# facebookresearch/metamorph

Measured on AMD Instinct MI355X. Metric: train tokens/sec (LLaMA-3-8B + SigLIP-SO400M, seq2048, 256 img toks), whole job, higher is better.
Workload: dtype bf16

## Files before the change

### include/mm355.h

```cpp
#ifndef MM355_H
#define MM355_H

#include <stddef.h>
#include <stdint.h>

#ifdef __cplusplus
extern "C" {
#endif

#define MM355_VERSION 100

#define MM355_OK            0
#define MM355_EINVAL       -1
#define MM355_EUNSUPPORTED -2
#define MM355_ELAUNCH      -3

typedef uint16_t mm355_bf16;

int mm355_version(void);
const char* mm355_strerror(int code);

#define MM355_GEMM_BIAS        1u
#define MM355_GEMM_GELU_ERF    2u
#define MM355_GEMM_GELU_TANH   4u
// ... 28 lines not shown
int mm355_gemm_rope_bf16(const mm355_bf16* X, int64_t ldx, const mm355_bf16* Wqkv, int64_t ldw, mm355_bf16* qkv, int64_t ld_qkv,
                         const mm355_bf16* cos_t, const mm355_bf16* sin_t, const int32_t* pos_offset,
                         int64_t M, int64_t N, int64_t K, int64_t L, int64_t n_rot, void* stream);

int mm355_gemm_swiglu_bwd_bf16(const mm355_bf16* dY, int64_t ldy, const mm355_bf16* WdT, int64_t ldw, const mm355_bf16* gu, int64_t ld_gu,
                               mm355_bf16* dgu, int64_t ld_dgu, mm355_bf16* actT, mm355_bf16* dguT, int64_t ldT,
                               int64_t M, int64_t I, int64_t K, void* stream);

int mm355_gemm_pair_bf16(const mm355_bf16* A0, int64_t lda0, const mm355_bf16* B0, int64_t ldb0, void* C0, int64_t ldc0,
                         int64_t M0, int64_t N0, int64_t K0, uint32_t flags0,
                         const mm355_bf16* A1, int64_t lda1, const mm355_bf16* B1, int64_t ldb1, void* C1, int64_t ldc1,
                         int64_t M1, int64_t N1, int64_t K1, uint32_t flags1, void* stream);

int mm355_transpose_bf16(const mm355_bf16* in, int64_t ld_in, int64_t rows, int64_t cols,
                         mm355_bf16* out, int64_t ld_out, void* stream);

int mm355_colsum_bf16(const mm355_bf16* dY, int64_t ld, int64_t M, int64_t N, float* db_f32, void* stream);

int mm355_rmsnorm_fwd(const mm355_bf16* x, const mm355_bf16* w, mm355_bf16* y, int64_t M, int64_t h,
                      float eps, void* stream);
int mm355_rmsnorm_fwd_rstd(const mm355_bf16* x, const mm355_bf16* w, mm355_bf16* y, float* rstd_out, int64_t M, int64_t h,
                           float eps, void* stream);
int mm355_rmsnorm_apply_t(const mm355_bf16* x, const mm355_bf16* w, const float* rstd, int64_t M, int64_t h,
                          mm355_bf16* out_t, int64_t ld_out, void* stream);
int mm355_rmsnorm_bwd(const mm355_bf16* dy, const mm355_bf16* x, const mm355_bf16* w,
                      const mm355_bf16* dres, mm355_bf16* dx, float* dw_f32, float* workspace,
                      int64_t M, int64_t h, float eps, void* stream);
int64_t mm355_rmsnorm_bwd_ws_floats(int64_t M, int64_t h);
int mm355_rmsnorm_bwd_wgrad(const mm355_bf16* dy, const mm355_bf16* x, const mm355_bf16* w, const mm355_bf16* dres,
                            mm355_bf16* dx, mm355_bf16* w_grad, int accumulate, float* workspace,
// ... 82 lines not shown
int mm355_swiglu_bwd_t(const mm355_bf16* gu, const mm355_bf16* dact, mm355_bf16* dgu, mm355_bf16* actT,
                       mm355_bf16* dguT, int64_t M, int64_t I, void* stream);
#define MM355_GELU_ERF  0
#define MM355_GELU_TANH 1
int mm355_gelu_fwd(const mm355_bf16* x, mm355_bf16* y, int64_t n, int kind, void* stream);
int mm355_gelu_bwd(const mm355_bf16* x, const mm355_bf16* dy, mm355_bf16* dx, int64_t n, int kind, void* stream);
int mm355_scale_bf16(mm355_bf16* x, int64_t n, const float* s_dev, float s_host, void* stream);
int mm355_axpy_bf16(mm355_bf16* y, const mm355_bf16* x, int64_t n, const float* s_dev, float s_host,
                    int accumulate, void* stream);
int mm355_axpy_f32_to_bf16(mm355_bf16* y, const float* x, int64_t n, float s_host, int accumulate, void* stream);
int mm355_axpy_f32_to_bf16_dev(mm355_bf16* y, const float* x, int64_t n, const float* s_dev, float s_host, int accumulate,
                               void* stream);

int mm355_ce_rows(mm355_bf16* logits, int64_t ld, const int32_t* targets, int64_t R, int64_t V,
                  float grad_scale, float* loss_sum, float* row_ws, void* stream);
int mm355_sum_rows_f32(const float* values, int64_t n, float scale, float* out, int accumulate, void* stream);

int64_t mm355_linear_ce_ws_bytes(int64_t n, int64_t V, int64_t h, int gather, int need_dh, int need_dw);
int mm355_linear_ce(const mm355_bf16* hidden, int64_t ldh, const int32_t* rows, const int32_t* targets, int64_t n,
                    const mm355_bf16* W, int64_t ldw, int64_t V, int64_t h, float* loss, mm355_bf16* d_hidden, void* dW,
                    int dw_f32, void* workspace, int64_t workspace_bytes, void* stream);

int mm355_splice_gather(const mm355_bf16* embed, const mm355_bf16* proj, const int32_t* src,
                        mm355_bf16* out, int64_t rows, int64_t h, void* stream);
int mm355_rows_gather(const mm355_bf16* in, int64_t ld_in, const int32_t* idx, mm355_bf16* out, int64_t ld_out,
                      int64_t R, int64_t h, void* stream);
int mm355_rows_scatter_add(const mm355_bf16* src, int64_t ld_src, const int32_t* idx, mm355_bf16* dst,
                           int64_t ld_dst, int64_t R, int64_t h, void* stream);
int mm355_embed_grad(const mm355_bf16* dout, const int32_t* tok, const int32_t* seg_start, const int32_t* pos,
                     int64_t n_seg, mm355_bf16* dembed, int64_t h, int accumulate, void* stream);
// ... 31 lines not shown
```

### metamorph_amd/csrc/gemm_bf16.hip

```cpp
#include "gemm_common.h"
#include <type_traits>
#include <cstdlib>

namespace {

template <int TM, int TN, int FM, int FN>
MM_DEV void gemm_epilogue(f32x4 (&acc)[FM][FN], const GemmArgs& a, unsigned char* smem, int m0, int n0, int wm, int wn, int wave, int lane) {
    const int fr = lane & 15, fq = lane >> 4;
    const int M = a.M, N = a.N;
    constexpr int CPL = TN / 4;
    float* stg = (float*)smem + wave * (16 * TN);
    const uint32_t fl = a.flags;
    const int row_l = lane >> 2, col_l = (lane & 3) * CPL;
    uint16_t* Cb = (uint16_t*)a.C;
    float* Cf = (float*)a.C;
    const bool vec_ok = ((a.ldc & 7) == 0) && (!(fl & MM355_GEMM_RESIDUAL) || (a.ldr & 7) == 0);
#pragma unroll
    for (int i = 0; i < FM; ++i) {
        __builtin_amdgcn_fence(__ATOMIC_RELEASE, "wavefront");
        __builtin_amdgcn_wave_barrier();
#pragma unroll
        for (int j = 0; j < FN; ++j)
#pragma unroll
            for (int r = 0; r < 4; ++r) stg[(fq * 4 + r) * TN + j * 16 + fr] = acc[i][j][r];
        __builtin_amdgcn_fence(__ATOMIC_RELEASE, "wavefront");
        __builtin_amdgcn_wave_barrier();
        const int grow = m0 + wm * TM + i * 16 + row_l;
        if (grow < M) {
            const int64_t rr = (fl & MM355_GEMM_RESIDUAL) ? (a.res_mod > 0 ? (int64_t)(grow % a.res_mod) : (int64_t)grow) : 0;
#pragma unroll
            for (int j = 0; j < CPL / 8; ++j) {
                const int c = n0 + wn * TN + col_l + j * 8;
                if (c >= N) continue;
                float v[8];
                const f32x4 s0 = *(const f32x4*)(stg + row_l * TN + col_l + j * 8);
                const f32x4 s1 = *(const f32x4*)(stg + row_l * TN + col_l + j * 8 + 4);
                v[0] = s0.x; v[1] = s0.y; v[2] = s0.z; v[3] = s0.w;
                v[4] = s1.x; v[5] = s1.y; v[6] = s1.z; v[7] = s1.w;
                epi_store8(a, fl, vec_ok, grow, rr, c, v);
            }
        }
    }
}

MM_DEV void gemm_epilogue_swiglu(f32x4 (&acc)[8][4], const GemmArgs& a, unsigned char* smem, int m0, int tn, int wm, int wn, int wave, int lane) {
    constexpr int TN = 64;
    const int fr = lane & 15, fq = lane >> 4;
    const int M = a.M, I = (int)a.res_mod;
    float* stg = (float*)smem + wave * (16 * TN);
    const int row_l = lane >> 2, k4 = lane & 3;
    uint16_t* gu = (uint16_t*)a.C;
    uint16_t* act = (uint16_t*)a.res;
    const int ch0 = tn * 128 + wn * 32;
#pragma unroll
// ... 383 lines not shown

template <int N> MM_DEV void wait_vmcnt() {
#if defined(MM355_SWB_ABL) && MM355_SWB_ABL == 3
    static_assert(N >= 0 && N <= 10, "unsupported count");
    asm volatile("s_waitcnt vmcnt(%0)" :: "n"(N) : "memory");
#else
    static_assert(N == 0 || N == 2 || N == 4 || N == 6 || N == 8, "unsupported count");
    if constexpr (N == 8) asm volatile("s_waitcnt vmcnt(8)" ::: "memory");
    else if constexpr (N == 6) asm volatile("s_waitcnt vmcnt(6)" ::: "memory");
    else if constexpr (N == 4) asm volatile("s_waitcnt vmcnt(4)" ::: "memory");
    else if constexpr (N == 2) asm volatile("s_waitcnt vmcnt(2)" ::: "memory");
    else asm volatile("s_waitcnt vmcnt(0)" ::: "memory");
#endif
}

template <int ABL = 0, bool SWI = false, bool SWB = false, bool ROPE = false>
MM_DEV void gemm_pp_tile(const GemmArgs& a, const int bid, unsigned char* smem) {
    constexpr int BM = 256, BN = 256, TM = 128, TN = 64, FM = 8, FN = 4;
    constexpr int BUF = (BM + BN) * 128;
    constexpr int A_BYTES = BM * 128;

    const int total = a.ntm * a.ntn;
    const int q8 = total >> 3, r8 = total & 7;
    const int xcd = bid & 7, idx = bid >> 3;
    const int logical = (xcd < r8 ? xcd * (q8 + 1) : r8 * (q8 + 1) + (xcd - r8) * q8) + idx;
    const int GM = a.gm;
    const int gsize = GM * a.ntn;
    const int grp = logical / gsize;
    const int first_m = grp * GM;
    const int gm = min(a.ntm - first_m, GM);
    const int in_g = logical - grp * gsize;
// ... 201 lines not shown
    __syncthreads();
#if defined(MM355_SWB_ABL) && (MM355_SWB_ABL == 1 || MM355_SWB_ABL == 3)
    if constexpr (SWB) {
        float keep = 0.f;
#pragma unroll
        for (int i = 0; i < FM; ++i)
#pragma unroll
            for (int j = 0; j < FN; ++j) keep += acc[i][j][0] + acc[i][j][1] + acc[i][j][2] + acc[i][j][3];
        if (keep == 1.2345e-30f) ((float*)a.C)[tid] = keep;
        return;
    }
#endif
    if constexpr (SWI) gemm_epilogue_swiglu(acc, a, smem, m0, tn, wm, wn, wave, lane);
    else if constexpr (SWB) gemm_epilogue_swiglu_bwd(acc, a, smem, m0, n0, wm, wn, wave, lane);
    else if constexpr (ROPE) gemm_epilogue_rope(acc, a, smem, m0, n0, wm, wn, wave, lane);
    else gemm_epilogue<TM, TN, FM, FN>(acc, a, smem, m0, n0, wm, wn, wave, lane);
}

__global__ __launch_bounds__(512) void gemm_pp_swiglu_kernel(GemmArgs a) {
    extern __shared__ __attribute__((aligned(16))) unsigned char smem[];
    gemm_pp_tile<0, true>(a, blockIdx.x, smem);
}

__global__ __launch_bounds__(512) void gemm_pp_rope_kernel(GemmArgs a) {
    extern __shared__ __attribute__((aligned(16))) unsigned char smem[];
    gemm_pp_tile<0, false, false, true>(a, blockIdx.x, smem);
}

__global__ __launch_bounds__(512) void gemm_pp_swiglu_bwd_kernel(GemmArgs a) {
    extern __shared__ __attribute__((aligned(16))) unsigned char smem[];
    gemm_pp_tile<0, false, true>(a, blockIdx.x, smem);
// ... 71 lines not shown
int launch_gemm(GemmArgs a, hipStream_t s) {
    constexpr int STAGE = (BM + BN) * 128;
    constexpr int LDS = 2 * STAGE;
    auto kern = gemm_nt_kernel<BM, BN, WM, WN, GLDS, PIPE>;
    static std::atomic<uint64_t> lds_ok{0};
    if (mm_ensure_dynamic_lds((const void*)kern, LDS, lds_ok) != MM355_OK) return MM355_ELAUNCH;
    a.ntm = (a.M + BM - 1) / BM;
    a.ntn = (a.N + BN - 1) / BN;
    const int64_t total = (int64_t)a.ntm * a.ntn;
    if (total <= 0 || total > 0x7fffffff) return MM355_EINVAL;
    hipLaunchKernelGGL(kern, dim3((unsigned)total), dim3(WM * WN * 64), LDS, s, a);
    return mm_launch_status();
}

__global__ __launch_bounds__(256) void transpose_kernel(const uint16_t* __restrict__ in, int64_t ld_in, int rows, int cols,
                                                        uint16_t* __restrict__ out, int64_t ld_out) {
    __shared__ uint16_t tile[64][64 + 2];
    const int r0 = blockIdx.y * 64, c0 = blockIdx.x * 64;
    const int tid = threadIdx.x;
#pragma unroll
    for (int i = 0; i < 2; ++i) {
        const int v = tid + i * 256, r = v >> 3, c = (v & 7) * 8;
        const int gr = r0 + r, gc = c0 + c;
        uint16_t tmp[8];
        if (gr < rows && gc + 8 <= cols) {
            *(u32x4*)tmp = *(const u32x4*)(in + (int64_t)gr * ld_in + gc);
        } else {
#pragma unroll
            for (int e = 0; e < 8; ++e) tmp[e] = (gr < rows && gc + e < cols) ? in[(int64_t)gr * ld_in + gc + e] : (uint16_t)0;
        }
#pragma unroll
        for (int e = 0; e < 8; ++e) tile[r][c + e] = tmp[e];
    }
    __syncthreads();
#pragma unroll
    for (int i = 0; i < 2; ++i) {
        const int v = tid + i * 256, c = v >> 3, r = (v & 7) * 8;
        const int gc = c0 + c, gr = r0 + r;
        if (gc >= cols) continue;
        uint16_t tmp[8];
#pragma unroll
        for (int e = 0; e < 8; ++e) tmp[e] = tile[r + e][c];
        if (gr + 8 <= rows && ((ld_out & 7) == 0)) {
            *(u32x4*)(out + (int64_t)gc * ld_out + gr) = *(const u32x4*)tmp;
        } else {
            for (int e = 0; e < 8; ++e)
                if (gr + e < rows) out[(int64_t)gc * ld_out + gr + e] = tmp[e];
        }
    }
}

__global__ __launch_bounds__(256) void colsum_kernel(const uint16_t* __restrict__ x, int64_t ld, int M, int N, float* __restrict__ out) {
    __shared__ float part[4][64];
    const int cq = threadIdx.x & 63, rp = threadIdx.x >> 6;
    const int c = blockIdx.x * 64 + cq;
    float s = 0.f;
    if (c < N)
        for (int r = rp; r < M; r += 4) s += bf2f(x[(int64_t)r * ld + c]);
    part[rp][cq] = s;
    __syncthreads();
    if (rp == 0 && c < N) out[c] += (part[0][cq] + part[1][cq]) + (part[2][cq] + part[3][cq]);
}
// ... 371 lines not shown
}

extern "C" int mm355_gemm_pair_bf16(const mm355_bf16* A0, int64_t lda0, const mm355_bf16* B0, int64_t ldb0, void* C0, int64_t ldc0,
                                    int64_t M0, int64_t N0, int64_t K0, uint32_t flags0,
                                    const mm355_bf16* A1, int64_t lda1, const mm355_bf16* B1, int64_t ldb1, void* C1, int64_t ldc1,
                                    int64_t M1, int64_t N1, int64_t K1, uint32_t flags1, void* stream) {
    (void)hipGetLastError();
    GemmArgs a0, a1;
    int rc = pair_problem(a0, A0, lda0, B0, ldb0, C0, ldc0, M0, N0, K0, flags0);
    if (rc != MM355_OK) return rc;
    rc = pair_problem(a1, A1, lda1, B1, ldb1, C1, ldc1, M1, N1, K1, flags1);
    if (rc != MM355_OK) return rc;
    return launch_gemm_pp_pair(a0, a1, (hipStream_t)stream);
}

extern "C" int mm355_transpose_bf16(const mm355_bf16* in, int64_t ld_in, int64_t rows, int64_t cols, mm355_bf16* out,
                                    int64_t ld_out, void* stream) {
    (void)hipGetLastError();
    if (!in || !out || rows <= 0 || cols <= 0 || (ld_in & 7) || !mm_aligned16(in) || !mm_aligned16(out)) return MM355_EINVAL;
    if (ld_out < rows || rows > 0x7fffffff || cols > 0x7fffffff) return MM355_EINVAL;
    dim3 grid((unsigned)((cols + 63) / 64), (unsigned)((rows + 63) / 64));
    hipLaunchKernelGGL(transpose_kernel, grid, dim3(256), 0, (hipStream_t)stream, in, ld_in, (int)rows, (int)cols, out, ld_out);
    return mm_launch_status();
}

extern "C" int mm355_gemm_swiglu_bf16(const mm355_bf16* X, int64_t ldx, const mm355_bf16* Wgu, int64_t ldw, mm355_bf16* gu, int64_t ld_gu,
                                      mm355_bf16* act, int64_t ld_act, int64_t M, int64_t I, int64_t K, void* stream) {
    (void)hipGetLastError();
    if (!X || !Wgu || !gu || !act || M <= 0 || I <= 0 || K <= 0) return MM355_EINVAL;
    if ((ldx & 7) || (ldw & 7) || (ld_gu & 7) || (ld_act & 7) || !mm_aligned16(X) || !mm_aligned16(Wgu) || !mm_aligned16(gu) || !mm_aligned16(act))
        return MM355_EINVAL;
    if (M > 0x7fffffff || I > 0x3fffffff || K > 0x7fffffff) return MM355_EINVAL;
    if ((I & 127) || K < 128 || (K & 127) || (2 * I * ldw + K) * 2 >= 0x7fffffffLL || (256 * ldx + K) * 2 >= 0x7fffffffLL) return MM355_EUNSUPPORTED;
    GemmArgs a = {};
    a.A = X; a.B = Wgu; a.C = gu; a.bias = nullptr; a.res = act;
    a.lda = ldx; a.ldb = ldw; a.ldc = ld_gu; a.ldr = ld_act; a.res_mod = I;
    a.M = (int)M; a.N = (int)(2 * I); a.K = (int)K; a.flags = 0; a.ntm = a.ntn = 0;
// ... 64 lines not shown
```

### metamorph_amd/csrc/linear_ce.hip

```cpp
#include "mm355_common.h"

#include <algorithm>

namespace {

constexpr int64_t CE_CHUNK = 8192;

inline int64_t up(int64_t x, int64_t a) { return (x + a - 1) / a * a; }
inline int64_t padded_rows(int64_t R) { return R >= 512 ? up(R, 128) : up(R, 8); }

struct Layout {
    int64_t Vp, chunk, rp, hc, wt, logits, dyT, xT, rows, total;
};

Layout layout(int64_t n, int64_t V, int64_t h, int gather, int need_dh, int need_dw) {
    Layout l{};
    l.Vp = up(V, 128);
    l.chunk = std::min(n, CE_CHUNK);
    l.rp = padded_rows(l.chunk);
    int64_t off = 0;
    auto take = [&](int64_t bytes) { const int64_t o = off; off += up(bytes, 256); return o; };
    l.hc = gather ? take(n * h * 2) : -1;
    l.wt = need_dh ? take(h * l.Vp * 2) : -1;
    l.logits = take(l.chunk * l.Vp * 2);
    l.dyT = need_dw ? take(V * l.rp * 2) : -1;
    l.xT = need_dw ? take(h * l.rp * 2) : -1;
    l.rows = take(n * 4);
    l.total = off;
    return l;
}

}

extern "C" int64_t mm355_linear_ce_ws_bytes(int64_t n, int64_t V, int64_t h, int gather, int need_dh, int need_dw) {
    if (n <= 0 || V <= 0 || h <= 0) return 0;
    return layout(n, V, h, gather, need_dh, need_dw).total;
}

extern "C" int mm355_linear_ce(const mm355_bf16* hidden, int64_t ldh, const int32_t* rows, const int32_t* targets, int64_t n,
                               const mm355_bf16* W, int64_t ldw, int64_t V, int64_t h, float* loss, mm355_bf16* d_hidden, void* dW,
                               int dw_f32, void* workspace, int64_t workspace_bytes, void* stream) {
    if (!hidden || !targets || !W || !loss || !workspace || n <= 0 || V <= 0 || h <= 0 || (h & 7) || (ldh & 7) || (ldw & 7) || ldh < h || ldw < h ||
        n > 0x7fffffff || !mm_aligned16(workspace))
        return MM355_EINVAL;
    const int need_dh = d_hidden != nullptr, need_dw = dW != nullptr, gather = rows != nullptr;
    const Layout l = layout(n, V, h, gather, need_dh, need_dw);
    if (workspace_bytes < l.total) return MM355_EINVAL;
    hipStream_t s = (hipStream_t)stream;
    char* ws = (char*)workspace;
    const mm355_bf16* hc = hidden;
    int64_t ldc = ldh;
    int rc;
    if (gather) {
        mm355_bf16* g = (mm355_bf16*)(ws + l.hc);
        if ((rc = mm355_rows_gather(hidden, ldh, rows, g, h, n, h, stream)) != MM355_OK) return rc;
        hc = g;
        ldc = h;
    }
    mm355_bf16* wt = need_dh ? (mm355_bf16*)(ws + l.wt) : nullptr;
    if (need_dh) {
        if (l.Vp != V && hipMemset2DAsync(wt + V, l.Vp * 2, 0, (l.Vp - V) * 2, h, s) != hipSuccess) return MM355_ELAUNCH;
        if ((rc = mm355_transpose_bf16(W, ldw, V, h, wt, l.Vp, stream)) != MM355_OK) return rc;
    }
    mm355_bf16* logits = (mm355_bf16*)(ws + l.logits);
    float* row_nll = (float*)(ws + l.rows);
    const float inv = 1.0f / (float)n;
    bool first = true;
    for (int64_t r0 = 0; r0 < n; r0 += CE_CHUNK) {
        const int64_t r = std::min(n - r0, CE_CHUNK);
        const mm355_bf16* x = hc + r0 * ldc;
        if ((rc = mm355_gemm_bf16(x, ldc, W, ldw, logits, l.Vp, r, V, h, nullptr, nullptr, 0, 0, 0u, 0, stream)) != MM355_OK) return rc;
        if ((rc = mm355_ce_rows(logits, l.Vp, targets + r0, r, V, inv, nullptr, row_nll + r0, stream)) != MM355_OK) return rc;
        if (need_dh &&
            (rc = mm355_gemm_bf16(logits, l.Vp, wt, l.Vp, d_hidden + r0 * h, h, r, h, l.Vp, nullptr, nullptr, 0, 0, 0u, 0, stream)) != MM355_OK)
            return rc;
        if (need_dw) {
            const int64_t rp = padded_rows(r);
            mm355_bf16* dyT = (mm355_bf16*)(ws + l.dyT);
            mm355_bf16* xT = (mm355_bf16*)(ws + l.xT);
            if (rp != r) {
                if (hipMemset2DAsync(dyT + r, rp * 2, 0, (rp - r) * 2, V, s) != hipSuccess) return MM355_ELAUNCH;
                if (hipMemset2DAsync(xT + r, rp * 2, 0, (rp - r) * 2, h, s) != hipSuccess) return MM355_ELAUNCH;
            }
            if ((rc = mm355_transpose_bf16(logits, l.Vp, r, V, dyT, rp, stream)) != MM355_OK) return rc;
            if ((rc = mm355_transpose_bf16(x, ldc, r, h, xT, rp, stream)) != MM355_OK) return rc;
            const uint32_t flags = (first ? 0u : MM355_GEMM_ACCUMULATE) | (dw_f32 ? MM355_GEMM_OUT_F32 : 0u);
            if ((rc = mm355_gemm_bf16(dyT, rp, xT, rp, dW, h, V, h, rp, nullptr, nullptr, 0, 0, flags, 0, stream)) != MM355_OK) return rc;
        }
        first = false;
    }
    return mm355_sum_rows_f32(row_nll, n, inv, loss, 0, stream);
}
```

### metamorph_amd/csrc/mm355_common.h

```cpp
#pragma once

#include <hip/hip_runtime.h>
#include <atomic>
#include <stdint.h>

#include "../../include/mm355.h"

typedef __attribute__((ext_vector_type(8))) short bf16x8;
typedef __attribute__((ext_vector_type(4))) short bf16x4;
typedef __attribute__((ext_vector_type(4))) float f32x4;
typedef __attribute__((ext_vector_type(16))) float f32x16;
typedef __attribute__((ext_vector_type(4))) uint32_t u32x4;
typedef __attribute__((ext_vector_type(2))) uint32_t u32x2;

#define MM_DEV __device__ __forceinline__

MM_DEV float bf2f(uint16_t h) { return __uint_as_float(((uint32_t)h) << 16); }
MM_DEV uint16_t f2bf(float f) {
    __bf16 b = (__bf16)f;
    return __builtin_bit_cast(uint16_t, b);
}
typedef float mm_f32x2 __attribute__((ext_vector_type(2)));
typedef __bf16 mm_bf16x2 __attribute__((ext_vector_type(2)));
MM_DEV uint32_t pack2bf(float lo, float hi) {
// ... 10 lines not shown
MM_DEV u32x4 pack8(const float* f) {
    u32x4 v;
    v.x = pack2bf(f[0], f[1]); v.y = pack2bf(f[2], f[3]); v.z = pack2bf(f[4], f[5]); v.w = pack2bf(f[6], f[7]);
    return v;
}

MM_DEV float wave_sum(float v) {
#pragma unroll
    for (int o = 32; o > 0; o >>= 1) v += __shfl_xor(v, o, 64);
    return v;
}
MM_DEV float wave_max(float v) {
#pragma unroll
    for (int o = 32; o > 0; o >>= 1) v = fmaxf(v, __shfl_xor(v, o, 64));
    return v;
}

template <int NT>
MM_DEV float block_sum(float v, float* red) {
    v = wave_sum(v);
    const int w = threadIdx.x >> 6, l = threadIdx.x & 63;
    __syncthreads();
    if (l == 0) red[w] = v;
    __syncthreads();
    float t = 0.f;
#pragma unroll
    for (int i = 0; i < NT / 64; ++i) t += red[i];
    return t;
}
template <int NT>
// ... 46 lines not shown
```

### metamorph_amd/csrc/rowwise.hip

```cpp
#include "mm355_common.h"
#include "rowsum.h"
#include <type_traits>

namespace {

constexpr int NT = 256;

template <int VPT>
__global__ __launch_bounds__(NT) void rmsnorm_fwd_kernel(const uint16_t* __restrict__ x, const uint16_t* __restrict__ w,
                                                         uint16_t* __restrict__ y, float* __restrict__ rstd_out, int h, float eps) {
    __shared__ float red[NT / 64];
    const int64_t row = blockIdx.x;
    const int nv = h >> 3;
    const uint16_t* xr = x + row * h;
    float xv[VPT][8];
    float ss = 0.f;
#pragma unroll
    for (int i = 0; i < VPT; ++i) {
        const int v = threadIdx.x + i * NT;
        if (v < nv) {
            unpack8(*(const u32x4*)(xr + v * 8), xv[i]);
#pragma unroll
            for (int e = 0; e < 8; ++e) ss += xv[i][e] * xv[i][e];
        }
// ... 308 lines not shown
        if (row_out) row_out[row] = lse - bf2f(lr[tgt]);
        else atomicAdd(loss_sum, lse - bf2f(lr[tgt]));
    }
    __syncthreads();
    for (int v = threadIdx.x; v < nvec; v += CE_NT) {
        float f[8];
        unpack8(*(const u32x4*)(lr + v * 8), f);
#pragma unroll
        for (int e = 0; e < 8; ++e) {
            const int c = v * 8 + e;
            float g = (c < V) ? __expf(f[e] - lse) : 0.f;
            if (c == tgt) g -= 1.0f;
            f[e] = g * grad_scale;
        }
        *(u32x4*)(lr + v * 8) = pack8(f);
    }
}

__global__ __launch_bounds__(NT) void cosine_loss_kernel(const uint16_t* __restrict__ pred, const uint16_t* __restrict__ tgt, int R, int C,
                                                         int normalize, float* __restrict__ cos_sum, uint16_t* __restrict__ dpred,
                                                         float* __restrict__ row_out) {
    const int row = blockIdx.x * (NT / 64) + (threadIdx.x >> 6);
    const int lane = threadIdx.x & 63;
    if (row >= R) return;
    const int nv = C >> 3;
    const uint16_t* pr = pred + (int64_t)row * C;
    const uint16_t* tr = tgt + (int64_t)row * C;
    float pp = 0.f;
    for (int v = lane; v < nv; v += 64) {
        float p[8];
// ... 343 lines not shown
    hipLaunchKernelGGL(mm_sum_rows_kernel, dim3(1), dim3(1024), 0, (hipStream_t)stream, values, n, scale, out, accumulate);
    return mm_launch_status();
}

extern "C" int mm355_ce_rows(mm355_bf16* logits, int64_t ld, const int32_t* targets, int64_t R, int64_t V, float grad_scale,
                             float* loss_sum, float* row_ws, void* stream) {
    (void)hipGetLastError();
    if (!logits || !targets || (!loss_sum && !row_ws) || R <= 0 || V <= 0 || ld < V || (ld & 7) || R > 0x7fffffff || !mm_aligned16(logits))
        return MM355_EINVAL;
    hipLaunchKernelGGL(ce_rows_kernel, dim3((unsigned)R), dim3(CE_NT), 0, (hipStream_t)stream, logits, ld, targets, (int)V, grad_scale, loss_sum,
                       row_ws);
    if (row_ws && loss_sum) hipLaunchKernelGGL(mm_sum_rows_kernel, dim3(1), dim3(1024), 0, (hipStream_t)stream, (const float*)row_ws, R, 1.0f, loss_sum, 1);
    return mm_launch_status();
}

extern "C" int mm355_cosine_loss(const mm355_bf16* pred_raw, const mm355_bf16* target, int64_t R, int64_t C, int normalize,
                                 float* cos_sum, mm355_bf16* dpred, float* row_ws, void* stream) {
    (void)hipGetLastError();
    if (!pred_raw || !target || !cos_sum || R <= 0 || C <= 0 || (C & 7)) return MM355_EINVAL;
    const unsigned grid = (unsigned)((R + NT / 64 - 1) / (NT / 64));
    hipLaunchKernelGGL(cosine_loss_kernel, dim3(grid), dim3(NT), 0, (hipStream_t)stream, pred_raw, target, (int)R, (int)C, normalize, cos_sum, dpred,
                       row_ws);
    if (row_ws) hipLaunchKernelGGL(mm_sum_rows_kernel, dim3(1), dim3(1024), 0, (hipStream_t)stream, (const float*)row_ws, R, 1.0f, cos_sum, 1);
    return mm_launch_status();
}

extern "C" int mm355_bilinear_l2norm_bwd(const mm355_bf16* in, const mm355_bf16* d_out, float* d_in_f32, int64_t N, int64_t side_in, int64_t side_out,
                                         int64_t C, int normalize, void* stream) {
    (void)hipGetLastError();
    if (!in || !d_out || !d_in_f32 || N <= 0 || side_in <= 0 || side_out <= 0 || C <= 0 || (C & 7)) return MM355_EINVAL;
// ... 17 lines not shown
```

### metamorph_amd/ops.py

```python
from __future__ import annotations

import os

import torch

from . import lib as _lib

BF16 = torch.bfloat16

GEMM_BIAS, GEMM_GELU_ERF, GEMM_GELU_TANH, GEMM_RESIDUAL, GEMM_ACCUMULATE, GEMM_OUT_F32 = 1, 2, 4, 8, 16, 32
GELU_ERF, GELU_TANH = 0, 1


def _L():
    return _lib.load()


def _stream():
    return torch.cuda.current_stream().cuda_stream


def _chk_dev(*ts):
    for t in ts:
        if t is not None and not t.is_cuda:
# ... 237 lines not shown


def transpose(x, out=None, ld_out=None):
    _chk_dev(x, out)
    px, R, C, ld = _rows2d(x)
    if out is None:
        ldo = ld_out or ((R + 7) // 8 * 8)
        buf = torch.empty((C, ldo), device=x.device, dtype=BF16)
        out = buf[:, :R]
    po, Co, Ro, ldo = _rows2d(out)
    assert Co == C and Ro == R
    _lib.check(_L().mm355_transpose_bf16(px, ld, R, C, po, ldo, _stream()), "mm355_transpose_bf16")
    return out


def colsum_f32(dy, out_f32):
    _chk_dev(dy, out_f32)
    p, M, N, ld = _rows2d(dy)
    assert out_f32.dtype == torch.float32 and out_f32.numel() >= N
    _lib.check(_L().mm355_colsum_bf16(p, ld, M, N, out_f32.data_ptr(), _stream()), "mm355_colsum_bf16")
    return out_f32



def rmsnorm_fwd(x, w, eps, out=None, want_rstd=False):
    _chk_dev(x, w)
    assert x.is_contiguous() and x.dtype == BF16 and w.dtype == BF16
    h = x.shape[-1]
    M = x.numel() // h
    out = torch.empty_like(x) if out is None else out
# ... 329 lines not shown
    return loss, dh, dw


def _row_ws(R, device, deterministic=True):
    return torch.empty((R,), device=device, dtype=torch.float32) if deterministic else None


def ce_rows_(logits2d, targets_i32, V, grad_scale, loss_sum_f32, deterministic=True):
    _chk_dev(logits2d, targets_i32, loss_sum_f32)
    p, R, _, ld = _rows2d(logits2d)
    assert targets_i32.dtype == torch.int32 and targets_i32.numel() >= R
    ws = _row_ws(R, logits2d.device, deterministic)
    _lib.check(_L().mm355_ce_rows(p, ld, targets_i32.data_ptr(), R, V, grad_scale, loss_sum_f32.data_ptr(), _p(ws), _stream()), "mm355_ce_rows")


def cosine_loss(pred_raw, target, normalize, want_grad=True):
    _chk_dev(pred_raw, target)
    assert pred_raw.is_contiguous() and target.is_contiguous() and pred_raw.shape == target.shape
    R, C = pred_raw.shape
    cos_sum = torch.zeros((1,), device=pred_raw.device, dtype=torch.float32)
    dpred = torch.empty_like(pred_raw) if want_grad else None
    _lib.check(_L().mm355_cosine_loss(pred_raw.data_ptr(), target.data_ptr(), R, C, int(normalize), cos_sum.data_ptr(), _p(dpred),
                                      _p(_row_ws(R, pred_raw.device)), _stream()), "mm355_cosine_loss")
    return cos_sum, dpred


def mean_abs_loss(pred, target, want_grad=True):
    _chk_dev(pred, target)
    assert pred.is_contiguous() and target.is_contiguous() and pred.shape == target.shape and pred.dtype == BF16 and target.dtype == BF16
    R, C = pred.shape
# ... 142 lines not shown
```

Baseline: 26740.

## Fuse CE row max/sum-exp into LM-head GEMM epilogue and gradient into transpose

The linear cross-entropy path now has the logits GEMM epilogue emit per-64-column slab (max, sum-exp) statistics. A small kernel combines these into a per-row logsumexp and NLL, which removes the separate full-row pass over the logits. A new grad kernel computes softmax gradients in place and writes the transposed dY with zero padding in the same pass, and transpose_pad replaces the memsets plus separate transposes. The cost is extra epilogue work in the GEMM, a stats workspace, and a fallback path for small grids.

After: 26740. No clear change (-0.0%).

```diff
diff --git a/include/mm355.h b/include/mm355.h
--- a/include/mm355.h
+++ b/include/mm355.h
@@ -66,6 +66,12 @@
 
 int mm355_transpose_bf16(const mm355_bf16* in, int64_t ld_in, int64_t rows, int64_t cols,
                          mm355_bf16* out, int64_t ld_out, void* stream);
+
+int mm355_transpose_pad_bf16(const mm355_bf16* in, int64_t ld_in, int64_t rows, int64_t cols,
+                             mm355_bf16* out, int64_t ld_out, int64_t rows_pad, void* stream);
+
+int mm355_gemm_rowstats_bf16(const mm355_bf16* A, int64_t lda, const mm355_bf16* B, int64_t ldb, mm355_bf16* C, int64_t ldc,
+                             int64_t M, int64_t N, int64_t K, float* stats, int64_t ld_stats, void* stream);
 
 int mm355_colsum_bf16(const mm355_bf16* dY, int64_t ld, int64_t M, int64_t N, float* db_f32, void* stream);
 
@@ -178,6 +184,11 @@
 
 int mm355_ce_rows(mm355_bf16* logits, int64_t ld, const int32_t* targets, int64_t R, int64_t V,
                   float grad_scale, float* loss_sum, float* row_ws, void* stream);
+int mm355_ce_slab_stats(const mm355_bf16* logits, int64_t ld, int64_t R, int64_t V, float* stats, int64_t ld_stats, void* stream);
+int mm355_ce_lse(const float* stats, int64_t ld_stats, const mm355_bf16* logits, int64_t ld, const int32_t* targets, int64_t R,
+                 int64_t V, float* lse, float* row_nll, void* stream);
+int mm355_ce_grad_t(mm355_bf16* logits, int64_t ld, const int32_t* targets, const float* lse, int64_t R, int64_t V,
+                    float grad_scale, mm355_bf16* dyT, int64_t ldT, int64_t Rp, void* stream);
 int mm355_sum_rows_f32(const float* values, int64_t n, float scale, float* out, int accumulate, void* stream);
 
 int64_t mm355_linear_ce_ws_bytes(int64_t n, int64_t V, int64_t h, int gather, int need_dh, int need_dw);
diff --git a/metamorph_amd/csrc/gemm_bf16.hip b/metamorph_amd/csrc/gemm_bf16.hip
--- a/metamorph_amd/csrc/gemm_bf16.hip
+++ b/metamorph_amd/csrc/gemm_bf16.hip
@@ -4,7 +4,7 @@
 
 namespace {
 
-template <int TM, int TN, int FM, int FN>
+template <int TM, int TN, int FM, int FN, bool STATS = false>
 MM_DEV void gemm_epilogue(f32x4 (&acc)[FM][FN], const GemmArgs& a, unsigned char* smem, int m0, int n0, int wm, int wn, int wave, int lane) {
     const int fr = lane & 15, fq = lane >> 4;
     const int M = a.M, N = a.N;
@@ -28,16 +28,37 @@
         const int grow = m0 + wm * TM + i * 16 + row_l;
         if (grow < M) {
             const int64_t rr = (fl & MM355_GEMM_RESIDUAL) ? (a.res_mod > 0 ? (int64_t)(grow % a.res_mod) : (int64_t)grow) : 0;
+            float f[STATS ? CPL : 1];
 #pragma unroll
             for (int j = 0; j < CPL / 8; ++j) {
                 const int c = n0 + wn * TN + col_l + j * 8;
-                if (c >= N) continue;
+                if (c >= N) {
+                    if constexpr (STATS) {
+#pragma unroll
+                        for (int e = 0; e < 8; ++e) f[j * 8 + e] = -INFINITY;
+                    }
+                    continue;
+                }
                 float v[8];
                 const f32x4 s0 = *(const f32x4*)(stg + row_l * TN + col_l + j * 8);
                 const f32x4 s1 = *(const f32x4*)(stg + row_l * TN + col_l + j * 8 + 4);
                 v[0] = s0.x; v[1] = s0.y; v[2] = s0.z; v[3] = s0.w;
                 v[4] = s1.x; v[5] = s1.y; v[6] = s1.z; v[7] = s1.w;
                 epi_store8(a, fl, vec_ok, grow, rr, c, v);
+                if constexpr (STATS) {
+                    unpack8(pack8(v), f + j * 8);
+                    if (n0 + wn * TN + TN > N) {
+#pragma unroll
+                        for (int e = 0; e < 8; ++e)
+                            if (c + e >= N) f[j * 8 + e] = -INFINITY;
+                    }
+                }
+            }
+            if constexpr (STATS) {
+                static_assert(!STATS || (TN == 64 && CPL == 16), "one slab = the 64 tile columns of a wave");
+                const mm_f32x2 ms = slab_stats16(f);
+                const int cs = n0 + wn * TN;
+                if ((lane & 3) == 0 && cs < N) ((mm_f32x2*)a.aux0)[(int64_t)(cs >> 6) * a.ld_aux + grow] = ms;
             }
         }
     }
@@ -451,7 +472,7 @@
 #endif
 }
 
-template <int ABL = 0, bool SWI = false, bool SWB = false, bool ROPE = false>
+template <int ABL = 0, bool SWI = false, bool SWB = false, bool ROPE = false, bool STATS = false>
 MM_DEV void gemm_pp_tile(const GemmArgs& a, const int bid, unsigned char* smem) {
     constexpr int BM = 256, BN = 256, TM = 128, TN = 64, FM = 8, FN = 4;
     constexpr int BUF = (BM + BN) * 128;
@@ -683,7 +704,12 @@
     if constexpr (SWI) gemm_epilogue_swiglu(acc, a, smem, m0, tn, wm, wn, wave, lane);
     else if constexpr (SWB) gemm_epilogue_swiglu_bwd(acc, a, smem, m0, n0, wm, wn, wave, lane);
     else if constexpr (ROPE) gemm_epilogue_rope(acc, a, smem, m0, n0, wm, wn, wave, lane);
-    else gemm_epilogue<TM, TN, FM, FN>(acc, a, smem, m0, n0, wm, wn, wave, lane);
+    else gemm_epilogue<TM, TN, FM, FN, STATS>(acc, a, smem, m0, n0, wm, wn, wave, lane);
+}
+
+__global__ __launch_bounds__(512) void gemm_pp_rowstats_kernel(GemmArgs a) {
+    extern __shared__ __attribute__((aligned(16))) unsigned char smem[];
+    gemm_pp_tile<0, false, false, false, true>(a, blockIdx.x, smem);
 }
 
 __global__ __launch_bounds__(512) void gemm_pp_swiglu_kernel(GemmArgs a) {
@@ -785,7 +811,7 @@
 }
 
 __global__ __launch_bounds__(256) void transpose_kernel(const uint16_t* __restrict__ in, int64_t ld_in, int rows, int cols,
-                                                        uint16_t* __restrict__ out, int64_t ld_out) {
+                                                        uint16_t* __restrict__ out, int64_t ld_out, int rows_out) {
     __shared__ uint16_t tile[64][64 + 2];
     const int r0 = blockIdx.y * 64, c0 = blockIdx.x * 64;
     const int tid = threadIdx.x;
@@ -812,11 +838,11 @@
         uint16_t tmp[8];
 #pragma unroll
         for (int e = 0; e < 8; ++e) tmp[e] = tile[r + e][c];
-        if (gr + 8 <= rows && ((ld_out & 7) == 0)) {
+        if (gr + 8 <= rows_out && ((ld_out & 7) == 0)) {
             *(u32x4*)(out + (int64_t)gc * ld_out + gr) = *(const u32x4*)tmp;
         } else {
             for (int e = 0; e < 8; ++e)
-                if (gr + e < rows) out[(int64_t)gc * ld_out + gr + e] = tmp[e];
+                if (gr + e < rows_out) out[(int64_t)gc * ld_out + gr + e] = tmp[e];
         }
     }
 }
@@ -1218,13 +1244,43 @@
     return launch_gemm_pp_pair(a0, a1, (hipStream_t)stream);
 }
 
+extern "C" int mm355_gemm_rowstats_bf16(const mm355_bf16* A, int64_t lda, const mm355_bf16* B, int64_t ldb, mm355_bf16* C, int64_t ldc,
+                                        int64_t M, int64_t N, int64_t K, float* stats, int64_t ld_stats, void* stream) {
+    (void)hipGetLastError();
+    if (!A || !B || !C || !stats || M <= 0 || N <= 0 || K <= 0 || ld_stats < M || ldc < N) return MM355_EINVAL;
+    if ((K & 7) || (lda & 7) || (ldb & 7) || !mm_aligned16(A) || !mm_aligned16(B) || !mm_aligned16(C) || (((uintptr_t)stats) & 7u)) return MM355_EINVAL;
+    if (M > 0x7fffffff || N > 0x7fffffff || K > 0x7fffffff) return MM355_EINVAL;
+    GemmArgs a = {};
+    a.A = A; a.B = B; a.C = C;
+    a.lda = lda; a.ldb = ldb; a.ldc = ldc;
+    a.M = (int)M; a.N = (int)N; a.K = (int)K;
+    a.aux0 = (uint16_t*)stats; a.ld_aux = ld_stats;
+    if (!pp_eligible(a)) return MM355_EUNSUPPORTED;
+    static std::atomic<uint64_t> lds_ok{0};
+    if (mm_ensure_dynamic_lds((const void*)gemm_pp_rowstats_kernel, PP_LDS, lds_ok) != MM355_OK) return MM355_ELAUNCH;
+    const int64_t total = pp_prepare(a);
+    if (total <= 0 || total > 0x7fffffff) return MM355_EINVAL;
+    hipLaunchKernelGGL(gemm_pp_rowstats_kernel, dim3((unsigned)total), dim3(512), PP_LDS, (hipStream_t)stream, a);
+    return mm_launch_status();
+}
+
 extern "C" int mm355_transpose_bf16(const mm355_bf16* in, int64_t ld_in, int64_t rows, int64_t cols, mm355_bf16* out,
                                     int64_t ld_out, void* stream) {
     (void)hipGetLastError();
     if (!in || !out || rows <= 0 || cols <= 0 || (ld_in & 7) || !mm_aligned16(in) || !mm_aligned16(out)) return MM355_EINVAL;
     if (ld_out < rows || rows > 0x7fffffff || cols > 0x7fffffff) return MM355_EINVAL;
     dim3 grid((unsigned)((cols + 63) / 64), (unsigned)((rows + 63) / 64));
-    hipLaunchKernelGGL(transpose_kernel, grid, dim3(256), 0, (hipStream_t)stream, in, ld_in, (int)rows, (int)cols, out, ld_out);
+    hipLaunchKernelGGL(transpose_kernel, grid, dim3(256), 0, (hipStream_t)stream, in, ld_in, (int)rows, (int)cols, out, ld_out, (int)rows);
+    return mm_launch_status();
+}
+
+extern "C" int mm355_transpose_pad_bf16(const mm355_bf16* in, int64_t ld_in, int64_t rows, int64_t cols, mm355_bf16* out,
+                                        int64_t ld_out, int64_t rows_pad, void* stream) {
+    (void)hipGetLastError();
+    if (!in || !out || rows <= 0 || cols <= 0 || (ld_in & 7) || !mm_aligned16(in) || !mm_aligned16(out)) return MM355_EINVAL;
+    if (rows_pad < rows || ld_out < rows_pad || rows_pad > 0x7fffffff || cols > 0x7fffffff) return MM355_EINVAL;
+    dim3 grid((unsigned)((cols + 63) / 64), (unsigned)((rows_pad + 63) / 64));
+    hipLaunchKernelGGL(transpose_kernel, grid, dim3(256), 0, (hipStream_t)stream, in, ld_in, (int)rows, (int)cols, out, ld_out, (int)rows_pad);
     return mm_launch_status();
 }
 
diff --git a/metamorph_amd/csrc/linear_ce.hip b/metamorph_amd/csrc/linear_ce.hip
--- a/metamorph_amd/csrc/linear_ce.hip
+++ b/metamorph_amd/csrc/linear_ce.hip
@@ -10,7 +10,7 @@
 inline int64_t padded_rows(int64_t R) { return R >= 512 ? up(R, 128) : up(R, 8); }
 
 struct Layout {
-    int64_t Vp, chunk, rp, hc, wt, logits, dyT, xT, rows, total;
+    int64_t Vp, chunk, rp, nslab, lds, hc, wt, logits, dyT, xT, stats, lse, rows, total;
 };
 
 Layout layout(int64_t n, int64_t V, int64_t h, int gather, int need_dh, int need_dw) {
@@ -25,6 +25,10 @@
     l.logits = take(l.chunk * l.Vp * 2);
     l.dyT = need_dw ? take(V * l.rp * 2) : -1;
     l.xT = need_dw ? take(h * l.rp * 2) : -1;
+    l.nslab = (V + 63) / 64;
+    l.lds = up(l.chunk, 16);
+    l.stats = take(l.nslab * l.lds * 8);
+    l.lse = take(l.chunk * 4);
     l.rows = take(n * 4);
     l.total = off;
     return l;
@@ -46,7 +50,6 @@
     const int need_dh = d_hidden != nullptr, need_dw = dW != nullptr, gather = rows != nullptr;
     const Layout l = layout(n, V, h, gather, need_dh, need_dw);
     if (workspace_bytes < l.total) return MM355_EINVAL;
-    hipStream_t s = (hipStream_t)stream;
     char* ws = (char*)workspace;
     const mm355_bf16* hc = hidden;
     int64_t ldc = ldh;
@@ -58,32 +61,36 @@
         ldc = h;
     }
     mm355_bf16* wt = need_dh ? (mm355_bf16*)(ws + l.wt) : nullptr;
-    if (need_dh) {
-        if (l.Vp != V && hipMemset2DAsync(wt + V, l.Vp * 2, 0, (l.Vp - V) * 2, h, s) != hipSuccess) return MM355_ELAUNCH;
-        if ((rc = mm355_transpose_bf16(W, ldw, V, h, wt, l.Vp, stream)) != MM355_OK) return rc;
-    }
+    if (need_dh &&
+        (rc = mm355_transpose_pad_bf16(W, ldw, V, h, wt, l.Vp, l.Vp, stream)) != MM355_OK)
+        return rc;
     mm355_bf16* logits = (mm355_bf16*)(ws + l.logits);
+    float* stats = (float*)(ws + l.stats);
+    float* lse = (float*)(ws + l.lse);
     float* row_nll = (float*)(ws + l.rows);
     const float inv = 1.0f / (float)n;
     bool first = true;
     for (int64_t r0 = 0; r0 < n; r0 += CE_CHUNK) {
         const int64_t r = std::min(n - r0, CE_CHUNK);
         const mm355_bf16* x = hc + r0 * ldc;
-        if ((rc = mm355_gemm_bf16(x, ldc, W, ldw, logits, l.Vp, r, V, h, nullptr, nullptr, 0, 0, 0u, 0, stream)) != MM355_OK) return rc;
-        if ((rc = mm355_ce_rows(logits, l.Vp, targets + r0, r, V, inv, nullptr, row_nll + r0, stream)) != MM355_OK) return rc;
+        rc = ((r + 255) / 256) * ((V + 255) / 256) >= 200 ? mm355_gemm_rowstats_bf16(x, ldc, W, ldw, logits, l.Vp, r, V, h, stats, l.lds, stream)
+                                                           : MM355_EUNSUPPORTED;
+        if (rc == MM355_EUNSUPPORTED) {
+            if ((rc = mm355_gemm_bf16(x, ldc, W, ldw, logits, l.Vp, r, V, h, nullptr, nullptr, 0, 0, 0u, 0, stream)) != MM355_OK) return rc;
+            rc = mm355_ce_slab_stats(logits, l.Vp, r, V, stats, l.lds, stream);
+        }
+        if (rc != MM355_OK) return rc;
+        if ((rc = mm355_ce_lse(stats, l.lds, logits, l.Vp, targets + r0, r, V, lse, row_nll + r0, stream)) != MM355_OK) return rc;
+        if (!need_dh && !need_dw) continue;
+        const int64_t rp = padded_rows(r);
+        mm355_bf16* dyT = need_dw ? (mm355_bf16*)(ws + l.dyT) : nullptr;
+        if ((rc = mm355_ce_grad_t(logits, l.Vp, targets + r0, lse, r, V, inv, dyT, rp, rp, stream)) != MM355_OK) return rc;
         if (need_dh &&
             (rc = mm355_gemm_bf16(logits, l.Vp, wt, l.Vp, d_hidden + r0 * h, h, r, h, l.Vp, nullptr, nullptr, 0, 0, 0u, 0, stream)) != MM355_OK)
             return rc;
         if (need_dw) {
-            const int64_t rp = padded_rows(r);
-            mm355_bf16* dyT = (mm355_bf16*)(ws + l.dyT);
             mm355_bf16* xT = (mm355_bf16*)(ws + l.xT);
-            if (rp != r) {
-                if (hipMemset2DAsync(dyT + r, rp * 2, 0, (rp - r) * 2, V, s) != hipSuccess) return MM355_ELAUNCH;
-                if (hipMemset2DAsync(xT + r, rp * 2, 0, (rp - r) * 2, h, s) != hipSuccess) return MM355_ELAUNCH;
-            }
-            if ((rc = mm355_transpose_bf16(logits, l.Vp, r, V, dyT, rp, stream)) != MM355_OK) return rc;
-            if ((rc = mm355_transpose_bf16(x, ldc, r, h, xT, rp, stream)) != MM355_OK) return rc;
+            if ((rc = mm355_transpose_pad_bf16(x, ldc, r, h, xT, rp, rp, stream)) != MM355_OK) return rc;
             const uint32_t flags = (first ? 0u : MM355_GEMM_ACCUMULATE) | (dw_f32 ? MM355_GEMM_OUT_F32 : 0u);
             if ((rc = mm355_gemm_bf16(dyT, rp, xT, rp, dW, h, V, h, rp, nullptr, nullptr, 0, 0, flags, 0, stream)) != MM355_OK) return rc;
         }
diff --git a/metamorph_amd/csrc/mm355_common.h b/metamorph_amd/csrc/mm355_common.h
--- a/metamorph_amd/csrc/mm355_common.h
+++ b/metamorph_amd/csrc/mm355_common.h
@@ -48,6 +48,22 @@
 #pragma unroll
     for (int o = 32; o > 0; o >>= 1) v = fmaxf(v, __shfl_xor(v, o, 64));
     return v;
+}
+
+MM_DEV mm_f32x2 slab_stats16(const float (&f)[16]) {
+    float m = f[0];
+#pragma unroll
+    for (int e = 1; e < 16; ++e) m = fmaxf(m, f[e]);
+    m = fmaxf(m, __shfl_xor(m, 1, 64));
+    m = fmaxf(m, __shfl_xor(m, 2, 64));
+    float s = 0.f;
+    if (m > -INFINITY) {
+#pragma unroll
+        for (int e = 0; e < 16; ++e) s += __expf(f[e] - m);
+    }
+    s += __shfl_xor(s, 1, 64);
+    s += __shfl_xor(s, 2, 64);
+    return mm_f32x2{m, s};
 }
 
 template <int NT>
diff --git a/metamorph_amd/csrc/rowwise.hip b/metamorph_amd/csrc/rowwise.hip
--- a/metamorph_amd/csrc/rowwise.hip
+++ b/metamorph_amd/csrc/rowwise.hip
@@ -346,6 +346,106 @@
             f[e] = g * grad_scale;
         }
         *(u32x4*)(lr + v * 8) = pack8(f);
+    }
+}
+
+__global__ __launch_bounds__(256) void ce_slab_stats_kernel(const uint16_t* __restrict__ logits, int64_t ld, int R, int V,
+                                                            mm_f32x2* __restrict__ stats, int64_t ld_stats) {
+    const int row = blockIdx.y * 64 + (threadIdx.x >> 2);
+    const int c0 = blockIdx.x * 64 + (threadIdx.x & 3) * 16;
+    if (row >= R) return;
+    float f[16];
+#pragma unroll
+    for (int j = 0; j < 2; ++j) {
+        const int c = c0 + j * 8;
+        if (c < V) {
+            unpack8(*(const u32x4*)(logits + (int64_t)row * ld + c), f + j * 8);
+#pragma unroll
+            for (int e = 0; e < 8; ++e)
+                if (c + e >= V) f[j * 8 + e] = -INFINITY;
+        } else {
+#pragma unroll
+            for (int e = 0; e < 8; ++e) f[j * 8 + e] = -INFINITY;
+        }
+    }
+    const mm_f32x2 ms = slab_stats16(f);
+    if ((threadIdx.x & 3) == 0) stats[(int64_t)blockIdx.x * ld_stats + row] = ms;
+}
+
+MM_DEV void ce_combine(float& m, float& s, const mm_f32x2 p) {
+    if (p.x > m) { s = s * __expf(m - p.x) + p.y; m = p.x; }
+    else if (p.x > -INFINITY) s += p.y * __expf(p.x - m);
+}
+
+__global__ __launch_bounds__(1024) void ce_lse_kernel(const mm_f32x2* __restrict__ stats, int64_t ld_stats, int nslab,
+                                                      const uint16_t* __restrict__ logits, int64_t ld, const int32_t* __restrict__ targets,
+                                                      int R, float* __restrict__ lse_out, float* __restrict__ row_out) {
+    __shared__ mm_f32x2 part[16][64];
+    const int rl = threadIdx.x & 63, ph = threadIdx.x >> 6;
+    const int row = blockIdx.x * 64 + rl;
+    float m = -INFINITY, s = 0.f;
+    if (row < R)
+        for (int sl = ph; sl < nslab; sl += 16) ce_combine(m, s, stats[(int64_t)sl * ld_stats + row]);
+    part[ph][rl] = mm_f32x2{m, s};
+    __syncthreads();
+    if (ph != 0 || row >= R) return;
+#pragma unroll
+    for (int i = 1; i < 16; ++i) ce_combine(m, s, part[i][rl]);
+    const int tgt = targets[row];
+    if (tgt < 0) {
+        lse_out[row] = INFINITY;
+        row_out[row] = 0.f;
+        return;
+    }
+    const float lse = m + __logf(s);
+    lse_out[row] = lse;
+    row_out[row] = lse - bf2f(logits[(int64_t)row * ld + tgt]);
+}
+
+__global__ __launch_bounds__(256) void ce_grad_t_kernel(uint16_t* __restrict__ logits, int64_t ld, const int32_t* __restrict__ targets,
+                                                        const float* __restrict__ lse, int R, int V, float grad_scale,
+                                                        uint16_t* __restrict__ dyT, int64_t ldT, int Rp) {
+    __shared__ uint16_t tile[64][64 + 2];
+    const int r0 = blockIdx.y * 64, c0 = blockIdx.x * 64;
+    const int tid = threadIdx.x;
+#pragma unroll
+    for (int i = 0; i < 2; ++i) {
+        const int v = tid + i * 256, r = v >> 3, c = (v & 7) * 8;
+        const int gr = r0 + r, gc = c0 + c;
+        uint16_t tmp[8];
+        *(u32x4*)tmp = u32x4{0u, 0u, 0u, 0u};
+        if (gr < R && gc < ld) {
+            uint16_t* p = logits + (int64_t)gr * ld + gc;
+            const int tgt = targets[gr];
+            const float l = lse[gr];
+            float f[8];
+            unpack8(*(const u32x4*)p, f);
+#pragma unroll
+            for (int e = 0; e < 8; ++e) {
+                const int cc = gc + e;
+                float g = (cc < V && tgt >= 0) ? __expf(f[e] - l) : 0.f;
+                if (cc == tgt) g -= 1.0f;
+                f[e] = g * grad_scale;
+            }
+            *(u32x4*)tmp = pack8(f);
+            *(u32x4*)p = *(const u32x4*)tmp;
+        }
+        if (dyT) {
+#pragma unroll
+            for (int e = 0; e < 8; ++e) tile[r][c + e] = tmp[e];
+        }
+    }
+    if (!dyT) return;
+    __syncthreads();
+#pragma unroll
+    for (int i = 0; i < 2; ++i) {
+        const int v = tid + i * 256, c = v >> 3, r = (v & 7) * 8;
+        const int gc = c0 + c, gr = r0 + r;
+        if (gc >= V || gr >= Rp) continue;
+        uint16_t tmp[8];
+#pragma unroll
+        for (int e = 0; e < 8; ++e) tmp[e] = tile[r + e][c];
+        *(u32x4*)(dyT + (int64_t)gc * ldT + gr) = *(const u32x4*)tmp;
     }
 }
 
@@ -719,6 +819,40 @@
     return mm_launch_status();
 }
 
+extern "C" int mm355_ce_slab_stats(const mm355_bf16* logits, int64_t ld, int64_t R, int64_t V, float* stats, int64_t ld_stats, void* stream) {
+    (void)hipGetLastError();
+    if (!logits || !stats || R <= 0 || V <= 0 || ld < V || (ld & 7) || R > 0x7fffffff || V > 0x7fffffff || ld_stats < R || !mm_aligned16(logits) ||
+        (((uintptr_t)stats) & 7u))
+        return MM355_EINVAL;
+    dim3 grid((unsigned)((V + 63) / 64), (unsigned)((R + 63) / 64));
+    hipLaunchKernelGGL(ce_slab_stats_kernel, grid, dim3(256), 0, (hipStream_t)stream, logits, ld, (int)R, (int)V, (mm_f32x2*)stats, ld_stats);
+    return mm_launch_status();
+}
+
+extern "C" int mm355_ce_lse(const float* stats, int64_t ld_stats, const mm355_bf16* logits, int64_t ld, const int32_t* targets, int64_t R,
+                            int64_t V, float* lse, float* row_nll, void* stream) {
+    (void)hipGetLastError();
+    if (!stats || !logits || !targets || !lse || !row_nll || R <= 0 || V <= 0 || ld < V || R > 0x7fffffff || V > 0x7fffffff || ld_stats < R ||
+        (((uintptr_t)stats) & 7u))
+        return MM355_EINVAL;
+    hipLaunchKernelGGL(ce_lse_kernel, dim3((unsigned)((R + 63) / 64)), dim3(1024), 0, (hipStream_t)stream, (const mm_f32x2*)stats, ld_stats,
+                       (int)((V + 63) / 64), logits, ld, targets, (int)R, lse, row_nll);
+    return mm_launch_status();
+}
+
+extern "C" int mm355_ce_grad_t(mm355_bf16* logits, int64_t ld, const int32_t* targets, const float* lse, int64_t R, int64_t V,
+                               float grad_scale, mm355_bf16* dyT, int64_t ldT, int64_t Rp, void* stream) {
+    (void)hipGetLastError();
+    if (!logits || !targets || !lse || R <= 0 || V <= 0 || ld < V || (ld & 7) || R > 0x7fffffff || ld > 0x7fffffff || !mm_aligned16(logits))
+        return MM355_EINVAL;
+    if (dyT && (Rp < R || (Rp & 7) || ldT < Rp || (ldT & 7) || Rp > 0x7fffffff || !mm_aligned16(dyT))) return MM355_EINVAL;
+    const int64_t rows = dyT ? Rp : R;
+    dim3 grid((unsigned)((ld + 63) / 64), (unsigned)((rows + 63) / 64));
+    hipLaunchKernelGGL(ce_grad_t_kernel, grid, dim3(256), 0, (hipStream_t)stream, logits, ld, targets, lse, (int)R, (int)V, grad_scale, dyT, ldT,
+                       (int)Rp);
+    return mm_launch_status();
+}
+
 extern "C" int mm355_cosine_loss(const mm355_bf16* pred_raw, const mm355_bf16* target, int64_t R, int64_t C, int normalize,
                                  float* cos_sum, mm355_bf16* dpred, float* row_ws, void* stream) {
     (void)hipGetLastError();
diff --git a/metamorph_amd/ops.py b/metamorph_amd/ops.py
--- a/metamorph_amd/ops.py
+++ b/metamorph_amd/ops.py
@@ -275,6 +275,15 @@
     return out
 
 
+def transpose_pad(x, out, rows_pad):
+    _chk_dev(x, out)
+    px, R, C, ld = _rows2d(x)
+    po, Co, Ro, ldo = _rows2d(out)
+    assert Co == C and Ro >= rows_pad >= R
+    _lib.check(_L().mm355_transpose_pad_bf16(px, ld, R, C, po, ldo, rows_pad, _stream()), "mm355_transpose_pad_bf16")
+    return out
+
+
 def colsum_f32(dy, out_f32):
     _chk_dev(dy, out_f32)
     p, M, N, ld = _rows2d(dy)
@@ -634,6 +643,54 @@
     _lib.check(_L().mm355_ce_rows(p, ld, targets_i32.data_ptr(), R, V, grad_scale, loss_sum_f32.data_ptr(), _p(ws), _stream()), "mm355_ce_rows")
 
 
+def gemm_rowstats(a, b, out, n=None):
+    _chk_dev(a, b, out)
+    pa, M, K, lda = _rows2d(a)
+    pb, N, Kb, ldb = _rows2d(b)
+    if n is not None:
+        N = n
+    po, Mo, No, ldc = _rows2d(out)
+    assert K == Kb and Mo == M and No >= N and a.dtype == BF16 and b.dtype == BF16 and out.dtype == BF16
+    lds = (M + 15) // 16 * 16
+    stats = torch.empty(((N + 63) // 64, lds, 2), device=a.device, dtype=torch.float32)
+    _lib.check(_L().mm355_gemm_rowstats_bf16(pa, lda, pb, ldb, po, ldc, M, N, K, stats.data_ptr(), lds, _stream()),
+               f"mm355_gemm_rowstats_bf16 M={M} N={N} K={K}")
+    return stats
+
+
+def ce_slab_stats(logits2d, V):
+    _chk_dev(logits2d)
+    p, R, _, ld = _rows2d(logits2d)
+    lds = (R + 15) // 16 * 16
+    stats = torch.empty(((V + 63) // 64, lds, 2), device=logits2d.device, dtype=torch.float32)
+    _lib.check(_L().mm355_ce_slab_stats(p, ld, R, V, stats.data_ptr(), lds, _stream()), "mm355_ce_slab_stats")
+    return stats
+
+
+def ce_lse(stats, logits2d, targets_i32, V):
+    _chk_dev(stats, logits2d, targets_i32)
+    p, R, _, ld = _rows2d(logits2d)
+    assert stats.dtype == torch.float32 and stats.is_contiguous() and stats.shape[0] == (V + 63) // 64 and stats.shape[1] >= R
+    assert targets_i32.dtype == torch.int32 and targets_i32.numel() >= R
+    lse = torch.empty((R,), device=logits2d.device, dtype=torch.float32)
+    nll = torch.empty((R,), device=logits2d.device, dtype=torch.float32)
+    _lib.check(_L().mm355_ce_lse(stats.data_ptr(), stats.shape[1], p, ld, targets_i32.data_ptr(), R, V, lse.data_ptr(), nll.data_ptr(),
+                                 _stream()), "mm355_ce_lse")
+    return lse, nll
+
+
+def ce_grad_t_(logits2d, targets_i32, lse, V, grad_scale, dyT=None, Rp=0):
+    _chk_dev(logits2d, targets_i32, lse, dyT)
+    p, R, _, ld = _rows2d(logits2d)
+    assert lse.dtype == torch.float32 and lse.numel() >= R and targets_i32.dtype == torch.int32 and targets_i32.numel() >= R
+    ldT = 0
+    if dyT is not None:
+        _, Vo, _, ldT = _rows2d(dyT)
+        assert Vo >= V and dyT.dtype == BF16
+    _lib.check(_L().mm355_ce_grad_t(p, ld, targets_i32.data_ptr(), lse.data_ptr(), R, V, grad_scale, _p(dyT), ldT, Rp, _stream()),
+               "mm355_ce_grad_t")
+
+
 def cosine_loss(pred_raw, target, normalize, want_grad=True):
     _chk_dev(pred_raw, target)
     assert pred_raw.is_contiguous() and target.is_contiguous() and pred_raw.shape == target.shape
```
